# taqu/cpprcoder

Hardware: AMD Instinct MI355X
Metric: MB/s encode+decode per GPU on 64 KiB blocks; ratio vs CPU ref (higher is better)
Workload: dtype u32

## Files before the change

cpprcoder_amd/csrc/rcx_api.hip:

```cpp
#include <hip/hip_runtime.h>

#include <cstdio>
#include <cstdlib>
#include <cstring>
#include <new>
#include <vector>

#include "../../include/rcx.h"
#include "rcx_divtab.hpp"
#include "rcx_kernels.hpp"

namespace
{

#define HIP_TRY(expr)                                                                                              \
    do {                                                                                                           \
        hipError_t e_ = (expr);                                                                                    \
        if (e_ != hipSuccess) {                                                                                    \
            if (getenv("RCX_DEBUG")) fprintf(stderr, "rcx: %s failed: %s (%s:%d)\n", #expr, hipGetErrorString(e_), __FILE__, __LINE__); \
            return RCX_E_HIP;                                                                                      \
        }                                                                                                          \
    } while (0)

struct EventPair {
    hipEvent_t a, b;
    int what;
};

inline hipError_t rcx_enter_device(int device)
{
    (void)hipGetLastError();
    return hipSetDevice(device);
}

struct HostPipe;

}

struct rcx_ctx {
    int device = 0;
    int lanes_per_block = 0;
    int wide_wg = -1;
    int enc_variant = 3;
    int enc_lanes = 0;
    int dec_quads = 0;
    int cus = 256;
    bool rans1_lds_set = false;
    bool rans1w_lds_set = false;
    bool rans_track = false;
    u8* slots = nullptr;
    u64 slots_bytes = 0;
    u32* sizes = nullptr;
    u64 sizes_count = 0;
    u32* starts = nullptr;
    u64 starts_count = 0;
    u32* models = nullptr;
    u64 models_bytes = 0;
    u32* redo = nullptr;
    u64 redo_count = 0;
    u32* ties = nullptr;
    u64 ties_count = 0;
    bool bwt_lds_set = false;
    bool bwt_atomic = false;
    DivEntry* divtab = nullptr;
    u32 divtab_block = 0;
    u32* status = nullptr;
    u32* status_host = nullptr;
    u8* h_in = nullptr;
    u64 h_in_bytes = 0;
    u8* h_out = nullptr;
    u64 h_out_bytes = 0;
    u64* h_off = nullptr;
    u64 h_off_count = 0;
    HostPipe* pipe = nullptr;
    bool timing = false;
    std::vector<EventPair> pending;
    std::vector<EventPair> pool;
    double ms[RCX_T_COUNT] = {};
    uint64_t launches[RCX_T_COUNT] = {};
};

namespace
{

struct Timed {
    rcx_ctx* c;
    hipStream_t s;
    EventPair p;
    bool on;
    Timed(rcx_ctx* ctx, hipStream_t st, int what) : c(ctx), s(st), on(ctx->timing)
    {
        if (!on) return;
        if (!c->pool.empty()) {
            p = c->pool.back();
            c->pool.pop_back();
        } else if (hipEventCreate(&p.a) != hipSuccess || hipEventCreate(&p.b) != hipSuccess) {
            on = false;
            return;
        }
        p.what = what;
        (void)hipEventRecord(p.a, s);
    }
    ~Timed()
    {
        if (!on) return;
        (void)hipEventRecord(p.b, s);
        c->pending.push_back(p);
    }
};

int grow(void** p, u64* have, u64 want)
{
    if (*have >= want) return RCX_OK;
    if (*p) (void)hipFree(*p);
    *p = nullptr;
    *have = 0;
    if (hipMalloc(p, want) != hipSuccess) return RCX_E_NOMEM;
    *have = want;
    return RCX_OK;
}

__global__ void rcx_divtab_k(DivEntry* __restrict__ tab, u64 entries)
{
    const u64 i = (u64)blockIdx.x * blockDim.x + threadIdx.x;
    if (i < entries) tab[i] = rcx_make_div_entry((u32)(256 + i));
}

int ensure_divtab(rcx_ctx* c, u32 block)
{
    if (c->divtab && c->divtab_block >= block) return RCX_OK;
    u32 cover = 1u << 16;
    while (cover < block) cover <<= 1;
    const u64 entries = (u64)cover + 2 * RCX_STAGE;
    if (c->divtab) (void)hipFree(c->divtab);
    c->divtab = nullptr;
    c->divtab_block = 0;
    if (hipMalloc(reinterpret_cast<void**>(&c->divtab), entries * sizeof(DivEntry)) != hipSuccess) return RCX_E_NOMEM;
    hipLaunchKernelGGL(rcx_divtab_k, dim3((u32)((entries + 255) / 256)), dim3(256), 0, nullptr, c->divtab, entries);
    if (hipGetLastError() != hipSuccess || hipDeviceSynchronize() != hipSuccess) return RCX_E_HIP;
    c->divtab_block = cover;
    return RCX_OK;
}

bool block_ok(uint32_t block) { return block >= RCX_MIN_BLOCK && block <= RCX_MAX_BLOCK; }

bool wide_workgroups(const rcx_ctx* c, u64 nblocks)
{
    (void)nblocks;
    return c->wide_wg != 0;
}

int decode_lanes(const rcx_ctx* c, u64 nblocks)
{
    (void)nblocks;
    return c->lanes_per_block ? c->lanes_per_block : 4;
}

u32 pow2_at_least(u64 x)
{
    u32 p = 1;
    while (p < x) p <<= 1;
    return p;
}
u32 encode_lanes(const rcx_ctx* c, u64 nblocks)
{
    if (c->enc_lanes) return (u32)c->enc_lanes;
    const u32 want = pow2_at_least((nblocks + c->cus - 1) / c->cus);
    return want > RCX_LANES ? RCX_LANES : want;
}
u32 decode_quads(const rcx_ctx* c, u64 nblocks)
{
    if (c->dec_quads) return (u32)c->dec_quads;
    const u64 simds = 4ull * c->cus;
    const u32 want = pow2_at_least((nblocks + simds - 1) / simds);
    return want > RCX_QUAD_BLOCKS ? RCX_QUAD_BLOCKS : want;
}

int ensure_redo(rcx_ctx* c, u64 nblocks)
{
    u64 bytes = c->redo_count * sizeof(u32);
    const int r = grow(reinterpret_cast<void**>(&c->redo), &bytes, (nblocks + 1) * sizeof(u32));
    c->redo_count = r == RCX_OK ? bytes / sizeof(u32) : 0;
    return r;
}

struct ScratchRange {
    u64 first = 0;
    bool packed = false;
};
struct ScratchView {
    u8* slots;
// ... 319 lines not shown
        if ((r = ensure_redo(c, nblocks)) != RCX_OK) return r;
    }
    return decode_range(c, coder, d_comp, comp_size, d_offsets, nblocks, block, n, d_dst, s, ScratchRange{});
}

}

namespace
{

int decode_range(rcx_ctx* c, int coder, const void* d_comp, u64 comp_size, const u64* d_offsets, u64 nblocks, u32 block, u64 n, void* d_dst,
                 hipStream_t s, ScratchRange rg)
{
    u32* const redo = c->redo ? c->redo + rg.first : nullptr;
    if (is_rans(coder)) {
        Timed t(c, s, RCX_T_DECODE);
        const u64 per_wg = 4 * RCX_RANS_BLOCKS;
        const u32 grid = (u32)((nblocks + per_wg - 1) / per_wg);
        if (coder == RCX_CODER_RANS8)
            hipLaunchKernelGGL(rcx_dec_rans8_k<4>, dim3(grid), dim3(256), 0, s, static_cast<const u8*>(d_comp), (u64)comp_size, d_offsets, nblocks,
                               block, n, static_cast<u8*>(d_dst), c->status);
        else {
            const u32 quads = rg.packed ? RCX_QUAD_BLOCKS : decode_quads(c, nblocks);
            const u64 per_wg1 = (u64)quads * RCX_QUAD_DEC_WAVES;
            const u32 grid1 = (u32)((nblocks + per_wg1 - 1) / per_wg1);
            hipLaunchKernelGGL(rcx_dec_rans1_quad_k<RCX_QUAD_DEC_WAVES>, dim3(grid1), dim3(64 * RCX_QUAD_DEC_WAVES), 0, s,
                               static_cast<const u8*>(d_comp), (u64)comp_size, d_offsets, nblocks, block, n, static_cast<u8*>(d_dst), c->status,
                               quads, c->rans_track ? c->status + 2 : static_cast<u32*>(nullptr));
        }
        return hipGetLastError() == hipSuccess ? RCX_OK : RCX_E_HIP;
    }
    const bool quad = coder == RCX_CODER_ADAPTIVE && decode_lanes(c, nblocks) == 4;
    const bool squad = coder == RCX_CODER_STATIC && decode_lanes(c, nblocks) != 1;
    {
        Timed t(c, s, RCX_T_DECODE);
        if (coder == RCX_CODER_STATIC && decode_lanes(c, nblocks) != 1) {
            const u32 quads = rg.packed ? RCX_QUAD_BLOCKS : decode_quads(c, nblocks);
            const u64 per_wg = (u64)quads * RCX_QUAD_DEC_WAVES;
            const u32 grid = (u32)((nblocks + per_wg - 1) / per_wg);
            hipLaunchKernelGGL(rcx_dec_static_quad_k<RCX_QUAD_DEC_WAVES>, dim3(grid), dim3(64 * RCX_QUAD_DEC_WAVES), 0, s,
                               static_cast<const u8*>(d_comp), (u64)comp_size, d_offsets, nblocks, block, n, static_cast<u8*>(d_dst), c->status,
                               redo, quads);
        } else if (coder == RCX_CODER_STATIC) {
            const u32 grid = (u32)((nblocks + RCX_LANES - 1) / RCX_LANES);
            hipLaunchKernelGGL(rcx_dec_static_k<false>, dim3(grid), dim3(64), 0, s, static_cast<const u8*>(d_comp), (u64)comp_size, d_offsets, nblocks,
                               block, n, static_cast<u8*>(d_dst), c->status, static_cast<u32*>(nullptr),
                               static_cast<const u32*>(nullptr));
        } else if (decode_lanes(c, nblocks) == 4) {
            const u32 quads = rg.packed ? RCX_QUAD_BLOCKS : decode_quads(c, nblocks);
            if (wide_workgroups(c, nblocks)) {
                const u64 per_wg = (u64)quads * RCX_QUAD_DEC_WAVES;
                const u32 grid = (u32)((nblocks + per_wg - 1) / per_wg);
                hipLaunchKernelGGL(rcx_dec_quad_k<RCX_QUAD_DEC_WAVES>, dim3(grid), dim3(64 * RCX_QUAD_DEC_WAVES), 0, s,
                                   static_cast<const u8*>(d_comp), (u64)comp_size, d_offsets, nblocks, block, n, static_cast<u8*>(d_dst), c->divtab,
                                   c->status, redo, quads);
            } else {
                const u32 grid = (u32)((nblocks + quads - 1) / quads);
                hipLaunchKernelGGL(rcx_dec_quad_k<1>, dim3(grid), dim3(64), 0, s, static_cast<const u8*>(d_comp), (u64)comp_size, d_offsets, nblocks,
                                   block, n, static_cast<u8*>(d_dst), c->divtab, c->status, redo, quads);
            }
#if defined(RCX_WITH_VARIANTS)
        } else if (decode_lanes(c, nblocks) == 8) {
            if (wide_workgroups(c, nblocks)) {
                const u64 per_wg = RCX_OCT_BLOCKS * RCX_OCT_DEC_WAVES;
                const u32 grid = (u32)((nblocks + per_wg - 1) / per_wg);
                hipLaunchKernelGGL(rcx_dec_oct_k<RCX_OCT_DEC_WAVES>, dim3(grid), dim3(64 * RCX_OCT_DEC_WAVES), 0, s,
                                   static_cast<const u8*>(d_comp), (u64)comp_size, d_offsets, nblocks, block, n, static_cast<u8*>(d_dst), c->divtab,
                                   c->status);
            } else {
                const u32 grid = (u32)((nblocks + RCX_OCT_BLOCKS - 1) / RCX_OCT_BLOCKS);
                hipLaunchKernelGGL(rcx_dec_oct_k<1>, dim3(grid), dim3(64), 0, s, static_cast<const u8*>(d_comp), (u64)comp_size, d_offsets, nblocks,
                                   block, n, static_cast<u8*>(d_dst), c->divtab, c->status);
            }
#endif
        } else {
            const u32 grid = (u32)((nblocks + RCX_LANES - 1) / RCX_LANES);
            hipLaunchKernelGGL(rcx_dec_adaptive_k<false>, dim3(grid), dim3(64), 0, s, static_cast<const u8*>(d_comp), (u64)comp_size, d_offsets,
                               nblocks, block, n, static_cast<u8*>(d_dst), c->divtab, c->status, static_cast<u32*>(nullptr),
                               static_cast<const u32*>(nullptr));
        }
        if (quad) {
            const u32 grid = (u32)((nblocks + RCX_LANES - 1) / RCX_LANES);
            hipLaunchKernelGGL(rcx_dec_adaptive_k<false>, dim3(grid), dim3(64), 0, s, static_cast<const u8*>(d_comp), (u64)comp_size, d_offsets,
                               nblocks, block, n, static_cast<u8*>(d_dst), c->divtab, c->status, static_cast<u32*>(nullptr),
                               static_cast<const u32*>(redo));
        }
        if (squad) {
            const u32 grid = (u32)((nblocks + RCX_LANES - 1) / RCX_LANES);
            hipLaunchKernelGGL(rcx_dec_static_k<false>, dim3(grid), dim3(64), 0, s, static_cast<const u8*>(d_comp), (u64)comp_size, d_offsets, nblocks,
                               block, n, static_cast<u8*>(d_dst), c->status, static_cast<u32*>(nullptr), static_cast<const u32*>(redo));
        }
    }
    return hipGetLastError() == hipSuccess ? RCX_OK : RCX_E_HIP;
}

}

extern "C" {

int rcx_encode_blocks(rcx_ctx* c, int coder, const uint8_t* src, uint64_t n, uint32_t block,
                      uint8_t* dst, uint64_t dst_cap, uint64_t* dst_size, uint64_t* offsets)
{
    if (!c || !block_ok(block) || !dst_size || (n && (!src || !dst))) return RCX_E_ARG;
    HIP_TRY(rcx_enter_device(c->device));
    *dst_size = 0;
    if (!coder_ok(coder)) return RCX_E_ARG;
    const u64 nblocks = rcx_block_count(n, block);
    if (nblocks > 0x7FFFFFFFull) return RCX_E_ARG;
    const u64 bound = rcx_encode_bound_for(coder, n, block);
    const u64 cb = host_chunk_blocks(block, false, nblocks);
    const u64 chunks = (nblocks + cb - 1) / cb;
    int r = grow(reinterpret_cast<void**>(&c->h_in), &c->h_in_bytes, n + 64);
// ... 317 lines not shown
            hipLaunchKernelGGL(rcx_dec_static_quad_k<RCX_QUAD_DEC_WAVES>, dim3(1), dim3(64 * RCX_QUAD_DEC_WAVES), 0, nullptr, c->h_in, (u64)comp_size,
                               c->h_off, (u64)1, block, count, c->h_out, c->status, c->redo, 1u);
            if (hipGetLastError() != hipSuccess) return RCX_E_HIP;
            u32 marked = 0;
            const int fast = rcx_ctx_sync_status(c, nullptr, nullptr);
            HIP_TRY(hipMemcpy(&marked, c->redo, sizeof(u32), hipMemcpyDeviceToHost));
            if (fast == RCX_OK && marked == 0) {
                HIP_TRY(hipMemcpy(dst, c->h_out, count, hipMemcpyDeviceToHost));
                *dst_size = count;
                return RCX_OK;
            }
        }
        hipLaunchKernelGGL(rcx_dec_static_k<true>, dim3(1), dim3(64), 0, nullptr, c->h_in, (u64)comp_size, c->h_off, (u64)1, block, count, c->h_out,
                           c->status, c->status + 2, static_cast<const u32*>(nullptr));
        if (hipGetLastError() != hipSuccess) return RCX_E_HIP;
        HIP_TRY(hipMemcpy(c->status_host, c->status, 4 * sizeof(u32), hipMemcpyDeviceToHost));
        const u32 short_at = c->status_host[2];
        const u64 produced = short_at < count ? short_at : count;
        if (produced) HIP_TRY(hipMemcpy(dst, c->h_out, produced, hipMemcpyDeviceToHost));
        *dst_size = produced;
        return short_at < count ? RCX_ERROR : RCX_OK;
    }
    if (comp_size < 8) {
        if (request_size) *request_size = 8;
        return RCX_PENDING;
    }
    const u32 declared = (u32)comp[0] | ((u32)comp[1] << 8) | ((u32)comp[2] << 16) | ((u32)comp[3] << 24);
    const u64 cap16 = sink_capacity;
    const u64 want = declared ? declared : 1;
    const u64 count = want < cap16 ? want : cap16;
    if (count > RCX_MAX_STREAM) return RCX_E_ARG;
    if (count == 0) {
        if (request_size) *request_size = declared;
        return RCX_PENDING;
    }
    const u32 block = count < RCX_MIN_BLOCK ? RCX_MIN_BLOCK : (u32)count;
    const bool longer = count > RCX_MAX_BLOCK;
    int r = longer ? RCX_OK : ensure_divtab(c, block);
    if (r != RCX_OK) return r;
    r = grow(reinterpret_cast<void**>(&c->h_in), &c->h_in_bytes, comp_size + 64);
    if (r != RCX_OK) return r;
    r = grow(reinterpret_cast<void**>(&c->h_out), &c->h_out_bytes, count + 64);
    if (r != RCX_OK) return r;
    u64 off_bytes = c->h_off_count * sizeof(u64);
    r = grow(reinterpret_cast<void**>(&c->h_off), &off_bytes, 2 * sizeof(u64));
    if (r != RCX_OK) return r;
    c->h_off_count = off_bytes / sizeof(u64);
    const u64 offs[2] = {0, comp_size};
    HIP_TRY(hipMemcpy(c->h_in, comp, comp_size, hipMemcpyHostToDevice));
    HIP_TRY(hipMemcpy(c->h_off, offs, sizeof(offs), hipMemcpyHostToDevice));
    if (!longer && count == declared && count >= RCX_MIN_BLOCK && decode_lanes(c, 1) == 4) {
        if ((r = ensure_redo(c, 1)) != RCX_OK) return r;
        hipLaunchKernelGGL(rcx_dec_quad_k<RCX_QUAD_DEC_WAVES>, dim3(1), dim3(64 * RCX_QUAD_DEC_WAVES), 0, nullptr, c->h_in, (u64)comp_size, c->h_off,
                           (u64)1, block, count, c->h_out, c->divtab, c->status, c->redo, 1u);
        if (hipGetLastError() != hipSuccess) return RCX_E_HIP;
        u32 marked = 0;
        const int fast = rcx_ctx_sync_status(c, nullptr, nullptr);
        HIP_TRY(hipMemcpy(&marked, c->redo, sizeof(u32), hipMemcpyDeviceToHost));
        if (fast == RCX_OK && marked == 0) {
            HIP_TRY(hipMemcpy(dst, c->h_out, count, hipMemcpyDeviceToHost));
            *dst_size = count;
            return RCX_OK;
        }
    }
    if (longer)
        hipLaunchKernelGGL((rcx_dec_adaptive_k<true, true>), dim3(1), dim3(64), 0, nullptr, c->h_in, (u64)comp_size, c->h_off, (u64)1, block, count, c->h_out,
                           c->divtab, c->status, c->status + 2, static_cast<const u32*>(nullptr));
    else
        hipLaunchKernelGGL((rcx_dec_adaptive_k<true, false>), dim3(1), dim3(64), 0, nullptr, c->h_in, (u64)comp_size, c->h_off, (u64)1, block, count, c->h_out,
                           c->divtab, c->status, c->status + 2, static_cast<const u32*>(nullptr));
    if (hipGetLastError() != hipSuccess) return RCX_E_HIP;
    HIP_TRY(hipMemcpy(c->status_host, c->status, 4 * sizeof(u32), hipMemcpyDeviceToHost));
    const u32 short_at = c->status_host[2];
    u64 produced = count;
    int result = RCX_OK;
    if (short_at != 0xFFFFFFFFu && short_at < count) {
        produced = short_at;
        result = RCX_PENDING;
    } else if (want > cap16) {
        result = RCX_PENDING;
    }
    if (result == RCX_PENDING && request_size) *request_size = declared - (u32)produced;
    if (produced) HIP_TRY(hipMemcpy(dst, c->h_out, produced, hipMemcpyDeviceToHost));
    *dst_size = produced;
    return result;
}

struct rcx_dstream {
    rcx_ctx* ctx = nullptr;
    RcxDState* state = nullptr;
    u8* in = nullptr;
    u64 in_base = 0;
    u64 in_bytes = 0, in_cap = 0;
    u64 consumed = 0;
    u8* out = nullptr;
    u32* result = nullptr;
    u32* result_host = nullptr;
    bool finished = false;
    u32 declared = 0, produced = 0;
};
#define RCX_DSTREAM_CHUNK (1u << 20)

int rcx_dstream_create(rcx_ctx* c, rcx_dstream** out)
{
    if (!c || !out) return RCX_E_ARG;
    *out = nullptr;
    HIP_TRY(rcx_enter_device(c->device));
// ... 507 lines not shown
```

cpprcoder_amd/csrc/rcx_oct.hpp:

```cpp
#pragma once

template <int CTRL>
__device__ __forceinline__ u32 rcx_dpp(u32 x)
{
    return (u32)__builtin_amdgcn_update_dpp(0, (int)x, CTRL, 0xF, 0xF, true);
}
__device__ __forceinline__ u32 rcx_oct_sum(u32 x)
{
    x += rcx_dpp<0xB1>(x);
    x += rcx_dpp<0x4E>(x);
    x += rcx_dpp<0x141>(x);
    return x;
}
__device__ __forceinline__ u32 rcx_oct_excl_scan(u32 x, u32 m1, u32 m2, u32 m4)
{
    u32 tot = x, pre = 0, o;
    o = rcx_dpp<0xB1>(tot);
    pre += o & m1;
    tot += o;
    o = rcx_dpp<0x4E>(tot);
    pre += o & m2;
    tot += o;
    o = rcx_dpp<0x141>(tot);
    pre += o & m4;
    return pre;
}

#define RCX_MC_CHUNK 16
#define RCX_MC_THREADS 256
#define RCX_MC_RING_U4 (2 * RCX_MC_CHUNK * RCX_LANES)
#define RCX_MC_LDS_U4 (RCX_LDS_U4 + RCX_MC_RING_U4)

__device__ __forceinline__ void rcx_lds_barrier()
{
    asm volatile("s_waitcnt lgkmcnt(0)\n\ts_barrier" ::: "memory");
}

#if defined(RCX_STAMP)
static __device__ unsigned long long rcx_stamp_out[16];
#define rcx_stamp_wait stamp_wait_
#endif
#define RCX_QUAD_BLOCKS 16
#define RCX_QUAD_STAGE 16
#define RCX_QUAD_GROUP_BYTES 4352
#define RCX_QUAD_RING_BYTES 144
#define RCX_QUAD_LDS_BYTES (RCX_QUAD_STAGE * 16 + 4 * RCX_QUAD_GROUP_BYTES + RCX_QUAD_BLOCKS * RCX_QUAD_RING_BYTES)

typedef u32 RcxV4 __attribute__((ext_vector_type(4)));
typedef __attribute__((address_space(3))) RcxV4 RcxLdsV4;
typedef __attribute__((address_space(3))) u32 RcxLdsU32;
typedef RcxV4 RcxDivQv;
typedef RcxLdsV4 RcxLdsDivQ;

struct alignas(16) DivQ {
    u32 mul, st;
    u64 add;
};

__device__ __forceinline__ u32 rcx_quad_sum(u32 x)
{
    x += rcx_dpp<0xB1>(x);
    x += rcx_dpp<0x4E>(x);
    return x;
}
__device__ __forceinline__ u32 rcx_umin(u32 a, u32 b) { return a < b ? a : b; }
__device__ __forceinline__ u32 rcx_umax(u32 a, u32 b) { return a > b ? a : b; }
__device__ __forceinline__ u32 rcx_quad_min(u32 x)
{
    x = rcx_umin(x, rcx_dpp<0xB1>(x));
    x = rcx_umin(x, rcx_dpp<0x4E>(x));
    return x;
}
__device__ __forceinline__ u32 rcx_quad_max(u32 x)
{
    x = rcx_umax(x, rcx_dpp<0xB1>(x));
    x = rcx_umax(x, rcx_dpp<0x4E>(x));
    return x;
}
__device__ __forceinline__ u32 rcx_quad_or(u32 x)
{
    x |= rcx_dpp<0xB1>(x);
    x |= rcx_dpp<0x4E>(x);
    return x;
}
__device__ __forceinline__ u32 rcx_quad_excl_scan(u32 x, u32 m1, u32 m2)
{
    u32 o = rcx_dpp<0xB1>(x);
    u32 pre = o & m1;
    const u32 tot = x + o;
    o = rcx_dpp<0x4E>(tot);
    pre += o & m2;
    return pre;
}

#if !defined(RCX_TOPUP_PIECES)
#define RCX_TOPUP_PIECES 1
#endif
struct QuadInput {
    u32 low, range;
    u32 bp8;
    u32 w0, w1;
    u32 n4;
    u32* ring;
    U4* skipped;
    u32 wr;
    u32 nfit;
    U4 pendA, pendB;
    const u8* origin;
    u32 last_off;
    u32 body8;
// ... 26 lines not shown
        origin = body - ((uintptr_t)body & 15);
        last_off = (u32)(stream_end - 1 - origin) & ~15u;
        wr = 0;
        for (u32 r = 0; r < 6; ++r) ring_put(load16(16 * r), true);
        nfit = 0;
        pendA.x = pendA.y = pendA.z = pendA.w = 0;
        pendB = pendA;
        body8 = 8u * (u32)(body - origin);
        bp8 = body8;
        fetch_pair();
        n4 = rcx_bswap(rcx_funnel_shr(w1, w0, bp8));
        return declared;
    }
    __device__ __forceinline__ void idle(const u8* anywhere, u32* block_ring, U4* scratch16)
    {
        skipped = scratch16;
        low = 0;
        range = 0x01000000u;
        ring = block_ring;
        origin = anywhere - ((uintptr_t)anywhere & 15);
        last_off = 0;
        wr = 24;
        nfit = 0;
        pendA.x = pendA.y = pendA.z = pendA.w = 0;
        pendB = pendA;
        body8 = bp8 = 0;
        w0 = w1 = n4 = 0;
    }
    __device__ __forceinline__ void topup()
    {
        ring_put(pendA, nfit >= 1);
#if RCX_TOPUP_PIECES > 1
        ring_put(pendB, nfit >= 2);
#endif
        const u32 rd = bp8 >> 5;
        if (rcx_any(wr - rd < 14u)) {
            asm volatile("" ::: "memory");
            while (__any(wr - rd <= 20u)) ring_put(load16(4 * wr), wr - rd <= 20u);
        }
        const u32 room = (rd + RCX_RING_DW - wr) >> 2;
        nfit = room < (u32)RCX_TOPUP_PIECES ? room : (u32)RCX_TOPUP_PIECES;
        pendA = load16(4 * wr);
#if RCX_TOPUP_PIECES > 1
        pendB = load16(4 * wr + 16);
#endif
    }
    __device__ __forceinline__ u64 taken() const { return 8 + (u64)((bp8 - body8) >> 3); }
};

#define RCX_QUAD_DEC_WAVES 4
template <int WAVES>
__global__ __launch_bounds__(64 * WAVES) void rcx_dec_quad_k(const u8* __restrict__ comp, u64 comp_size, const u64* __restrict__ offsets,
                                                             u64 nblocks, u32 block, u64 n, u8* __restrict__ dst,
                                                             const DivEntry* __restrict__ divtab, u32* status,
                                                             u32* __restrict__ redo, u32 quads_used)
{
    __shared__ __attribute__((aligned(256))) u8 lds_all[WAVES * RCX_QUAD_LDS_BYTES];
    const u32 lane = threadIdx.x & 63u;
    const u32 wave_in_wg = __builtin_amdgcn_readfirstlane(threadIdx.x >> 6);
    u8* lds = lds_all + wave_in_wg * RCX_QUAD_LDS_BYTES;
    const u32 j = lane & 3u, quad = lane >> 2;
    const bool in_use = quad < quads_used;
    const u64 blk = ((u64)blockIdx.x * WAVES + wave_in_wg) * quads_used + (quad & (quads_used - 1u));
    bool live = blk < nblocks;
    const u64 at = live ? blk * (u64)block : 0;
    u32 len = live ? (u32)((n - at) < (u64)block ? (n - at) : (u64)block) : 0u;

    DivQ* stage = reinterpret_cast<DivQ*>(lds);
    const u32 group = 2u * (quad >> 3) + ((0x96u >> (quad & 7u)) & 1u), quarter = (quad & 7u) >> 1;
    u8* mine = lds + RCX_QUAD_STAGE * 16 + group * RCX_QUAD_GROUP_BYTES + quarter * 64;
    U4* leaves = reinterpret_cast<U4*>(mine) + j;
    U4* parked = reinterpret_cast<U4*>(mine + 16 * 256);
    u32* block_ring = reinterpret_cast<u32*>(lds + RCX_QUAD_STAGE * 16 + 4 * RCX_QUAD_GROUP_BYTES + quad * RCX_QUAD_RING_BYTES);
    {
        U4 v;
        v.x = v.y = v.z = v.w = 1;
#pragma unroll
        for (u32 q = 0; q < 17; ++q) leaves[q * 16] = v;
    }
    u32 U1 = 64u * j + 16, U2 = U1 + 16, U3 = U1 + 32, U4_ = U1 + 48;
    const u32 T0 = 4u * j;
    const u32 m1 = (j & 1u) ? ~0u : 0u, m2 = (j & 2u) ? ~0u : 0u;

    QuadInput in;
    u64 stream_len = 0;
    if (live) {
        const u64 s0 = offsets[blk], s1 = offsets[blk + 1];
        stream_len = s1 - s0;
        if (s1 < s0 || s1 > comp_size || stream_len < 9) {
            if (j == 0 && in_use) rcx_flag(status, RCX_ST_CORRUPT, blk);
            live = false;
            len = 0;
        } else {
            const u32 declared = in.begin(comp + s0, comp + s1, block_ring, parked + 3);
            if (declared != len) {
                if (j == 0 && in_use) rcx_flag(status, RCX_ST_CORRUPT, blk);
                live = false;
                len = 0;
            }
        }
    }
    if (!live) in.idle(comp, block_ring, parked + 3);

    const u32 maxlen = rcx_wave_max(len);
    u8* out = dst + at;
    u32 fast_end;
    {
        u32 mine = live ? (len & ~15u) : 0xFFFFFFF0u;
        if (live && (reinterpret_cast<uintptr_t>(out) & 15u) != 0) mine = 0;
#pragma unroll
        for (int o = 32; o > 0; o >>= 1) {
            const u32 other = (u32)__shfl_xor((int)mine, o, 64);
            mine = mine < other ? mine : other;
        }
        fast_end = mine == 0xFFFFFFF0u ? 0u : mine;
    }
    const bool leader = live && in_use && j == 0;

    const u32 T0p3 = T0 + 3;
    const u32 leaves_lds = (u32)reinterpret_cast<uintptr_t>(leaves);
    const u32 ring_lds = (u32)reinterpret_cast<uintptr_t>(block_ring);
#if defined(RCX_STAMP_DEC)
#define RCX_QUAD_STAMP(i) if (stamp_now_) stamp_t_[stamp_at_ + (i)] = __builtin_amdgcn_s_memtime();
#else
#define RCX_QUAD_STAMP(i)
#endif
#define RCX_QP1 "quad_perm:[1,0,3,2] row_mask:0xf bank_mask:0xf bound_ctrl:1\n\t"
#define RCX_QP2 "quad_perm:[2,3,0,1] row_mask:0xf bank_mask:0xf bound_ctrl:1\n\t"
    u32 p_sym_ = 0, p_la_ = leaves_lds;
    u64 p_own_ = 0;
#define RCX_QD_PREV_A_0 "s_nop 1\n\t"
#define RCX_QD_PREV_A_1 "v_cndmask_b32_e64 %[pown], 0, 1, %[pc]\n\t"                                                \
                        "v_and_b32 %[pad], 3, %[psym]\n\t"                                                         \
                        "v_lshl_add_u32 %[pad], %[pad], 2, %[pla]\n\t"
#define RCX_QD_PREV_S_0
#define RCX_QD_PREV_S_1 "\n\tv_cndmask_b32_e64 %[pye], 0, %[psym], %[pc]\n\t"                                       \
                        "v_lshl_or_b32 %[pword], %[pye], %[psh], %[pword]"
#define RCX_QUAD_DEC_SYMBOL(K, HP, PWORD, PSHIFT)                                                           \
    {                                                                                                      \
            \
        const u32 k8_ = rcx_clz(in.range) & 0x18u;                                                         \
        in.low = (u32)((((u64)in.low << 32) | in.n4) << k8_ >> 32);                                        \
        in.range <<= k8_;                                                                                  \
        const DivQ k_ = (K);                                                                               \
        const u32 t_ = (u32)(((u64)in.range * k_.mul + k_.add) >> 32) >> (k_.st & 31u);           \
              \
        const u32 a1_ = rcx_mul24(U1, t_), a2_ = rcx_mul24(U2, t_), a3_ = rcx_mul24(U3, t_);               \
        const u32 a4_ = rcx_mul24(U4_, t_);                                                                \
        u32 node_, rem_, ro_, la_, x1_, x2_, x3_, x4_, pown_, pad_, pye_;                                  \
        u64 c1_, c2_, c3_, c4_, cz_;                                                                       \
        asm volatile("v_sub_co_u32_e64 %[x1], %[c1], %[low], %[a1]\n\t"                                    \
                     "v_sub_co_u32_e64 %[x2], %[c2], %[low], %[a2]\n\t"                                    \
                     "v_sub_co_u32_e64 %[x3], %[c3], %[low], %[a3]\n\t"                                    \
                     "v_sub_co_u32_e64 %[x4], %[c4], %[low], %[a4]\n\t"                                    \
                     "v_subb_co_u32_e64 %[nd], %[cz], 4, 0, %[c1]\n\t"  \
                     "v_subb_co_u32_e64 %[nd], %[cz], %[nd], 0, %[c2]\n\t"                                 \
                     "v_subb_co_u32_e64 %[nd], %[cz], %[nd], 0, %[c3]\n\t"                                 \
                     "v_subb_co_u32_e64 %[nd], %[cz], %[nd], 0, %[c4]\n\t"                                 \
                     RCX_QD_PREV_A_##HP                                                                    \
                     : [nd] "=&v"(node_), [x1] "=&v"(x1_), [x2] "=&v"(x2_), [x3] "=&v"(x3_), [x4] "=&v"(x4_), \
                       [c1] "=&s"(c1_), [c2] "=&s"(c2_), [c3] "=&s"(c3_), [c4] "=&s"(c4_), [cz] "=&s"(cz_), \
                       [pown] "=&v"(pown_), [pad] "=&v"(pad_)                                              \
                     : [low] "v"(in.low), [a1] "v"(a1_), [a2] "v"(a2_), [a3] "v"(a3_), [a4] "v"(a4_),      \
                       [pc] "s"(p_own_), [psym] "v"(p_sym_), [pla] "v"(p_la_));                            \
        if (HP) (void)__hip_atomic_fetch_add(reinterpret_cast<RcxLdsU32*>(pad_), pown_, __ATOMIC_RELAXED, __HIP_MEMORY_SCOPE_WAVEFRONT);  \
        asm volatile("v_add_u32_dpp %[nd], %[nd], %[nd] " RCX_QP1                                          \
                     "v_add_u32 %[bp], %[bp], %[k8]\n\t"                 \
                     "v_bfe_u32 %[ro], %[bp], 5, 5\n\t"                 \
                     "v_lshl_add_u32 %[ro], %[ro], 2, %[rb]"  \
                     : [nd] "+v"(node_), [ro] "=&v"(ro_), [bp] "+v"(in.bp8)                                 \
                     : [k8] "v"(k8_), [rb] "v"(ring_lds));                                                 \
        {                                                                                                  \
            const RcxLdsU32* at_ = reinterpret_cast<const RcxLdsU32*>(ro_);  \
            in.w0 = at_[0];                                                                                \
            in.w1 = at_[1];                                                                                \
        }                                                                                                  \
        __builtin_amdgcn_sched_barrier(0);                                                                 \
        asm volatile("v_add_u32_dpp %[nd], %[nd], %[nd] " RCX_QP2                                          \
                     "v_lshl_add_u32 %[la], %[nd], 8, %[lvb]"  \
                     : [nd] "+v"(node_), [la] "=&v"(la_)                                                    \
                     : [lvb] "v"(leaves_lds));                                                             \
                                                              \
        RCX_QUAD_STAMP(0);                                                                                 \
        const RcxV4 l_ = *reinterpret_cast<const RcxLdsV4*>(la_);                                          \
        __builtin_amdgcn_sched_barrier(0);                                                                 \
                    \
        u32 sb_;                                                                                           \
        asm volatile("v_min3_u32 %[rm], %[x1], %[x2], %[x3]\n\t"                                           \
                     "v_min3_u32 %[rm], %[rm], %[x4], %[low]\n\t"                                          \
                     "v_addc_co_u32_e64 %[u1], %[c1], 0, %[u1], %[c1]\n\t"                                 \
                     "v_addc_co_u32_e64 %[u2], %[c2], 0, %[u2], %[c2]\n\t"                                 \
                     "v_min_u32_dpp %[rm], %[rm], %[rm] " RCX_QP1                                          \
                     "v_addc_co_u32_e64 %[u3], %[c3], 0, %[u3], %[c3]\n\t"                                 \
                     "v_addc_co_u32_e64 %[u4], %[c4], 0, %[u4], %[c4]\n\t"                                 \
                     "v_min_u32_dpp %[rm], %[rm], %[rm] " RCX_QP2                                          \
                     "v_lshl_add_u32 %[sb], %[n], 4, %[t0p3]"  \
                     RCX_QD_PREV_S_##HP                                                                    \
                     : [u1] "+v"(U1), [u2] "+v"(U2), [u3] "+v"(U3), [u4] "+v"(U4_), [rm] "=&v"(rem_),       \
// ... 5 lines not shown
        asm volatile("v_mul_u32_u24 %[qa], %[lx], %[t]\n\t"       \
                     "v_mad_u32_u24 %[qb], %[ly], %[t], %[qa]\n\t"       \
                     "v_mad_u32_u24 %[qc], %[lz], %[t], %[qb]\n\t"                                         \
                     "v_mad_u32_u24 %[qe], %[lw], %[t], %[qc]\n\t"                                         \
                     "v_alignbit_b32 %[n4], %[w1], %[w0], %[bp]\n\t"  \
                     "v_perm_b32 %[n4], %[n4], %[n4], %[swap]\n\t"  \
                     "v_add_u32_dpp %[tot], %[qe], %[qe] " RCX_QP1  \
                     "v_and_b32_dpp %[pre], %[qe], %[m1] " RCX_QP1                                         \
                     "v_sub_u32 %[d2], %[rem], %[pre]\n\t"                                                 \
                     "v_and_b32_dpp %[o2], %[tot], %[m2] " RCX_QP2                                         \
                     "v_sub_u32 %[d2], %[d2], %[o2]\n\t"      \
                     "v_sub_co_u32_e64 %[ya], %[c1], %[d2], %[qa]\n\t"                                     \
                     "v_sub_co_u32_e64 %[yb], %[c2], %[d2], %[qb]\n\t"                                     \
                     "v_sub_co_u32_e64 %[yc], %[c3], %[d2], %[qc]\n\t"                                     \
                     "v_sub_co_u32_e64 %[ye], %[own], %[d2], %[qe]\n\t"  \
                     "v_min3_u32 %[lo], %[d2], %[ya], %[yb]\n\t"                                           \
                     "v_max3_u32 %[hi], %[ya], %[yb], %[yc]\n\t"                                           \
                     "v_min_u32 %[lo], %[lo], %[yc]\n\t"                                                   \
                     "v_max_u32 %[hi], %[hi], %[ye]\n\t"                                                   \
                     "v_subb_co_u32_e64 %[sym], %[c1], %[sb], 0, %[c1]\n\t"                                \
                     "v_min_u32_dpp %[lo], %[lo], %[lo] " RCX_QP1                                          \
                     "v_subb_co_u32_e64 %[sym], %[c2], %[sym], 0, %[c2]\n\t"                               \
                     "v_max_u32_dpp %[hi], %[hi], %[hi] " RCX_QP1                                          \
                     "v_subb_co_u32_e64 %[sym], %[c3], %[sym], 0, %[c3]\n\t"                               \
                     "v_min_u32_dpp %[lo], %[lo], %[lo] " RCX_QP2                                          \
                     "v_max_u32_dpp %[hi], %[hi], %[hi] " RCX_QP2                                          \
                     "v_sub_u32 %[rg], %[lo], %[hi]"                                                       \
                     : [lo] "=&v"(lo_), [rg] "=&v"(rg_), [sym] "=&v"(p_sym_), [own] "=&s"(p_own_), [n4] "=&v"(in.n4), \
                       [qa] "=&v"(qa_), [qb] "=&v"(qb_), [qc] "=&v"(qc_),                                   \
                       [qe] "=&v"(qe_), [tot] "=&v"(tot_), [pre] "=&v"(pre_), [o2] "=&v"(o2_), [d2] "=&v"(d2_), \
                       [ya] "=&v"(ya_), [yb] "=&v"(yb_), [yc] "=&v"(yc_), [ye] "=&v"(ye_), [hi] "=&v"(hi_),  \
                       [c1] "=&s"(c1_), [c2] "=&s"(c2_), [c3] "=&s"(c3_)                                   \
                     : [lx] "v"(l_.x), [ly] "v"(l_.y), [lz] "v"(l_.z), [lw] "v"(l_.w), [t] "v"(t_),        \
                       [rem] "v"(rem_), [m1] "v"(m1), [m2] "v"(m2), [sb] "v"(sb_),                         \
                       [w0] "v"(in.w0), [w1] "v"(in.w1), [bp] "v"(in.bp8), [swap] "s"(0x00010203u));       \
        RCX_QUAD_STAMP(1);                                                                                 \
        in.low = lo_;                                                                            \
        in.range = rg_;                                                                          \
        p_la_ = la_;                                                                                       \
    }
#define RCX_QUAD_DEC_FINISH(WORD, SHIFT)                                                                    \
    {                                                                                                      \
        u32 pown_, pad_, pye_;                                                                             \
        asm volatile("v_cndmask_b32_e64 %[pown], 0, 1, %[pc]\n\t"                                          \
                     "v_and_b32 %[pad], 3, %[psym]\n\t"                                                    \
                     "v_cndmask_b32_e64 %[pye], 0, %[psym], %[pc]\n\t"                                     \
                     "v_lshl_add_u32 %[pad], %[pad], 2, %[pla]\n\t"                                        \
                     "v_lshl_or_b32 %[pword], %[pye], %[psh], %[pword]"                                    \
                     : [pown] "=&v"(pown_), [pad] "=&v"(pad_), [pye] "=&v"(pye_), [pword] "+v"(WORD)        \
                     : [pc] "s"(p_own_), [psym] "v"(p_sym_), [pla] "v"(p_la_), [psh] "n"(SHIFT));          \
        (void)__hip_atomic_fetch_add(reinterpret_cast<RcxLdsU32*>(pad_), pown_, __ATOMIC_RELAXED, __HIP_MEMORY_SCOPE_WAVEFRONT);  \
    }

    DivEntry ahead = divtab[lane % RCX_QUAD_STAGE];
#define RCX_QUAD_STAGE_PUT()                                                                               \
    {                                                                                                      \
        DivQ q_;                                                                                           \
        q_.mul = ahead.mul;                                                                                \
        q_.st = (ahead.total << 5) | ahead.shift;                                                          \
        q_.add = ahead.add;                                                                                \
        stage[lane % RCX_QUAD_STAGE] = q_;                           \
    }
#define RCX_QUAD_STAGE_GET(I0) ahead = divtab[(I0) + RCX_QUAD_STAGE + lane % RCX_QUAD_STAGE];
    {
        U4 o_last;
        o_last.x = o_last.y = o_last.z = o_last.w = 0;
#if defined(RCX_STAMP_DEC)
        unsigned long long stamp_sum_[4] = {0, 0, 0, 0};
#endif
        for (u32 i0 = 0; i0 < fast_end; i0 += 16) {
            RCX_QUAD_STAGE_PUT();
            in.topup();
            RCX_QUAD_STAGE_GET(i0);
            const u32 g = (i0 >> 4) & 3u;
            if (g == 0 && i0 != 0 && leader) {
                U4* o4 = reinterpret_cast<U4*>(out + (i0 - 64));
                const U4 p0 = parked[0], p1 = parked[1], p2 = parked[2];
                o4[0] = p0;
                o4[1] = p1;
                o4[2] = p2;
                o4[3] = o_last;
            }
            u32 w0_ = 0, w1_ = 0, w2_ = 0, w3_ = 0;
            DivQ k_next = stage[0];
#if defined(RCX_STAMP_DEC)
            unsigned long long stamp_t_[4] = {0, 0, 0, 0};
#define RCX_QUAD_STEP(S, HP, PW)                                 \
    {                                                            \
        const DivQ kk = k_next;                                  \
        if ((S) + 1 < 16) k_next = stage[(S) + 1];               \
        const bool stamp_now_ = (S) == 8 || (S) == 9;            \
        const int stamp_at_ = (S) == 8 ? 0 : 2;                  \
        RCX_QUAD_DEC_SYMBOL(kk, HP, PW, (8 * (((S) + 3) & 3))); \
    }
#else
#define RCX_QUAD_STEP(S, HP, PW)                                 \
    {                                                            \
        const DivQ kk = k_next;                                  \
        if ((S) + 1 < 16) k_next = stage[(S) + 1];               \
        RCX_QUAD_DEC_SYMBOL(kk, HP, PW, (8 * (((S) + 3) & 3))); \
    }
#endif
            RCX_QUAD_STEP(0, 0, w0_) RCX_QUAD_STEP(1, 1, w0_) RCX_QUAD_STEP(2, 1, w0_) RCX_QUAD_STEP(3, 1, w0_)
            RCX_QUAD_STEP(4, 1, w0_) RCX_QUAD_STEP(5, 1, w1_) RCX_QUAD_STEP(6, 1, w1_) RCX_QUAD_STEP(7, 1, w1_)
            RCX_QUAD_STEP(8, 1, w1_) RCX_QUAD_STEP(9, 1, w2_) RCX_QUAD_STEP(10, 1, w2_) RCX_QUAD_STEP(11, 1, w2_)
            RCX_QUAD_STEP(12, 1, w2_) RCX_QUAD_STEP(13, 1, w3_) RCX_QUAD_STEP(14, 1, w3_) RCX_QUAD_STEP(15, 1, w3_)
            RCX_QUAD_DEC_FINISH(w3_, 24)
#undef RCX_QUAD_STEP
#if defined(RCX_STAMP_DEC)
            stamp_sum_[0] += stamp_t_[1] - stamp_t_[0];
            stamp_sum_[1] += stamp_t_[2] - stamp_t_[1];
            stamp_sum_[2] += stamp_t_[3] - stamp_t_[2];
            stamp_sum_[3] += 1;
#endif
            U4 o;
            o.x = rcx_quad_or(w0_);
            o.y = rcx_quad_or(w1_);
            o.z = rcx_quad_or(w2_);
            o.w = rcx_quad_or(w3_);
            if (g == 3) o_last = o;
            else parked[g] = o;
        }
#if defined(RCX_STAMP_DEC)
        if (blockIdx.x == 7 && threadIdx.x == 0)
            for (int i_ = 0; i_ < 4; ++i_) rcx_dec_stamp_out[i_] = stamp_sum_[i_];
#endif
        if (leader && fast_end != 0) {
            const u32 groups = ((fast_end - 1) >> 4 & 3u) + 1;
            U4* o4 = reinterpret_cast<U4*>(out + ((fast_end - 1) & ~63u));
            o4[0] = parked[0];
            if (groups > 1) o4[1] = parked[1];
            if (groups > 2) o4[2] = parked[2];
            if (groups > 3) o4[3] = o_last;
        }
    }
    {
        for (u32 i = fast_end; i < maxlen; ++i) {
            if ((i & 15u) == 0) {
                RCX_QUAD_STAGE_PUT();
                in.topup();
                RCX_QUAD_STAGE_GET(i);
            }
            const DivQ k = stage[i % RCX_QUAD_STAGE];
            if (i < len) {
                u32 part = 0;
#if defined(RCX_STAMP_DEC)
                const bool stamp_now_ = false;
                const int stamp_at_ = 0;
                unsigned long long stamp_t_[4];
#endif
                RCX_QUAD_DEC_SYMBOL(k, 0, part, 0);
                RCX_QUAD_DEC_FINISH(part, 0);
                part = rcx_quad_or(part);
                if (leader) out[i] = (u8)part;
            }
        }
    }
#undef RCX_QUAD_DEC_SYMBOL
#undef RCX_QUAD_DEC_FINISH
#undef RCX_QD_PREV_A_0
#undef RCX_QD_PREV_A_1
#undef RCX_QD_PREV_S_0
#undef RCX_QD_PREV_S_1
#undef RCX_QUAD_STAGE_PUT
#undef RCX_QUAD_STAGE_GET
#undef RCX_QP1
#undef RCX_QP2
    const bool marked = live && rcx_quad_or(j == 3 && U4_ != 256u + len ? 1u : 0u) != 0;
    if (leader && !marked && in.taken() > stream_len) rcx_flag(status, RCX_ST_CORRUPT, blk);
    if (leader) redo[blk] = marked ? 1u : 0u;
    else if (j == 0 && in_use && blk < nblocks) redo[blk] = 0;
}

#if !defined(RCX_DRAIN_WAVE)
#define RCX_DRAIN_WAVE 5
#endif
#if RCX_DRAIN_WAVE == 5
#define RCX_MC5_THREADS 384
#define RCX_MC5_ROLE(HW) ((HW) == 1u ? 3u : (HW) == 3u ? 1u : (HW))
#else
#define RCX_MC5_THREADS 320
#define RCX_MC5_ROLE(HW) (HW)
#endif
#if !defined(RCX_RING_PLANAR)
#define RCX_RING_PLANAR 0
#endif
#if !defined(RCX_MODEL_AHEAD)
#define RCX_MODEL_AHEAD 2
#endif
#if !defined(RCX_ARITH_AHEAD)
#define RCX_ARITH_AHEAD 1
#endif
#if RCX_RING_PLANAR
#define RCX_RING_LANE 1
#define RCX_RING_AT(s, f) ((4 * (s) + (f)) * RCX_LANES)
#else
#define RCX_RING_LANE 4
#define RCX_RING_AT(s, f) (4 * (s) * RCX_LANES + (f))
#endif
#define RCX_MC5_RING2_DW (2 * RCX_MC_CHUNK * RCX_LANES)
#define RCX_OUT_RING_WORDS 64
#define RCX_OUT_MARGIN 32
#define RCX_MC5_OUT_DW (RCX_OUT_RING_WORDS * RCX_LANES + 3 * RCX_LANES)
#define RCX_MC5_LDS_U4 (RCX_MC_LDS_U4 + RCX_MC5_RING2_DW / 4 + RCX_LANES / 4 + RCX_MC5_OUT_DW / 4)

struct __attribute__((packed, aligned(4))) RcxU4Unaligned {
    u32 x, y, z, w;
};

__device__ __attribute__((noinline, cold)) u32 rcx_stage_carry(u32* ring_lane, u32 pos, u32 safe_from, u32 extra)
{
    while (extra != 0 && pos > safe_from) {
        --pos;
        u32* w = ring_lane + ((pos >> 2) % RCX_OUT_RING_WORDS) * RCX_LANES;
        const u32 sh = 8u * (pos & 3u);
        const u32 old = *w;
        const u32 v = ((old >> sh) & 0xFFu) + extra;
        *w = (old & ~(0xFFu << sh)) | ((v & 0xFFu) << sh);
// ... 418 lines not shown
```

Before: 69560.

## Replace LDS-staged division table with packed global mul/inc table in quad decoder

Adds a second precomputed table holding each divisor's multiplier and a 0/1 increment flag, packed in groups of 16 so a quad can load four U4 vectors per 16-symbol group. The quad decoder now computes the quotient with __umulhi((range<<k)+inc, mul) >> shift, with the shift derived from clz of the position, instead of a 64-bit multiply-add. The LDS staging area and its per-group store and reload are removed, and loads for the next group are software-pipelined between steps. This trades LDS traffic and 64-bit arithmetic for global/scalar loads held in extra registers, and relies on the increment formulation matching the old add term exactly.

```diff
diff --git a/cpprcoder_amd/csrc/rcx_api.hip b/cpprcoder_amd/csrc/rcx_api.hip
--- a/cpprcoder_amd/csrc/rcx_api.hip
+++ b/cpprcoder_amd/csrc/rcx_api.hip
@@ -63,6 +63,7 @@
     bool bwt_lds_set = false;
     bool bwt_atomic = false;
     DivEntry* divtab = nullptr;
+    u32* divq = nullptr;
     u32 divtab_block = 0;
     u32* status = nullptr;
     u32* status_host = nullptr;
@@ -120,10 +121,16 @@
     return RCX_OK;
 }
 
-__global__ void rcx_divtab_k(DivEntry* __restrict__ tab, u64 entries)
+__global__ void rcx_divtab_k(DivEntry* __restrict__ tab, u32* __restrict__ divq, u64 entries)
 {
     const u64 i = (u64)blockIdx.x * blockDim.x + threadIdx.x;
-    if (i < entries) tab[i] = rcx_make_div_entry((u32)(256 + i));
+    if (i < entries) {
+        const DivEntry e = rcx_make_div_entry((u32)(256 + i));
+        tab[i] = e;
+        u32* g = divq + (i >> 4) * RCX_QUAD_DIVQ_DW + (i & 15u);
+        g[0] = e.mul;
+        g[16] = e.add == 0 ? 0u : 1u;
+    }
 }
 
 int ensure_divtab(rcx_ctx* c, u32 block)
@@ -134,9 +141,11 @@
     const u64 entries = (u64)cover + 2 * RCX_STAGE;
     if (c->divtab) (void)hipFree(c->divtab);
     c->divtab = nullptr;
+    c->divq = nullptr;
     c->divtab_block = 0;
-    if (hipMalloc(reinterpret_cast<void**>(&c->divtab), entries * sizeof(DivEntry)) != hipSuccess) return RCX_E_NOMEM;
-    hipLaunchKernelGGL(rcx_divtab_k, dim3((u32)((entries + 255) / 256)), dim3(256), 0, nullptr, c->divtab, entries);
+    if (hipMalloc(reinterpret_cast<void**>(&c->divtab), entries * (sizeof(DivEntry) + 2 * sizeof(u32))) != hipSuccess) return RCX_E_NOMEM;
+    c->divq = reinterpret_cast<u32*>(c->divtab + entries);
+    hipLaunchKernelGGL(rcx_divtab_k, dim3((u32)((entries + 255) / 256)), dim3(256), 0, nullptr, c->divtab, c->divq, entries);
     if (hipGetLastError() != hipSuccess || hipDeviceSynchronize() != hipSuccess) return RCX_E_HIP;
     c->divtab_block = cover;
     return RCX_OK;
@@ -562,12 +571,12 @@
                 const u64 per_wg = (u64)quads * RCX_QUAD_DEC_WAVES;
                 const u32 grid = (u32)((nblocks + per_wg - 1) / per_wg);
                 hipLaunchKernelGGL(rcx_dec_quad_k<RCX_QUAD_DEC_WAVES>, dim3(grid), dim3(64 * RCX_QUAD_DEC_WAVES), 0, s,
-                                   static_cast<const u8*>(d_comp), (u64)comp_size, d_offsets, nblocks, block, n, static_cast<u8*>(d_dst), c->divtab,
+                                   static_cast<const u8*>(d_comp), (u64)comp_size, d_offsets, nblocks, block, n, static_cast<u8*>(d_dst), c->divq,
                                    c->status, redo, quads);
             } else {
                 const u32 grid = (u32)((nblocks + quads - 1) / quads);
                 hipLaunchKernelGGL(rcx_dec_quad_k<1>, dim3(grid), dim3(64), 0, s, static_cast<const u8*>(d_comp), (u64)comp_size, d_offsets, nblocks,
-                                   block, n, static_cast<u8*>(d_dst), c->divtab, c->status, redo, quads);
+                                   block, n, static_cast<u8*>(d_dst), c->divq, c->status, redo, quads);
             }
 #if defined(RCX_WITH_VARIANTS)
         } else if (decode_lanes(c, nblocks) == 8) {
@@ -991,7 +1000,7 @@
     if (!longer && count == declared && count >= RCX_MIN_BLOCK && decode_lanes(c, 1) == 4) {
         if ((r = ensure_redo(c, 1)) != RCX_OK) return r;
         hipLaunchKernelGGL(rcx_dec_quad_k<RCX_QUAD_DEC_WAVES>, dim3(1), dim3(64 * RCX_QUAD_DEC_WAVES), 0, nullptr, c->h_in, (u64)comp_size, c->h_off,
-                           (u64)1, block, count, c->h_out, c->divtab, c->status, c->redo, 1u);
+                           (u64)1, block, count, c->h_out, c->divq, c->status, c->redo, 1u);
         if (hipGetLastError() != hipSuccess) return RCX_E_HIP;
         u32 marked = 0;
         const int fast = rcx_ctx_sync_status(c, nullptr, nullptr);
diff --git a/cpprcoder_amd/csrc/rcx_oct.hpp b/cpprcoder_amd/csrc/rcx_oct.hpp
--- a/cpprcoder_amd/csrc/rcx_oct.hpp
+++ b/cpprcoder_amd/csrc/rcx_oct.hpp
@@ -41,10 +41,9 @@
 #define rcx_stamp_wait stamp_wait_
 #endif
 #define RCX_QUAD_BLOCKS 16
-#define RCX_QUAD_STAGE 16
 #define RCX_QUAD_GROUP_BYTES 4352
 #define RCX_QUAD_RING_BYTES 144
-#define RCX_QUAD_LDS_BYTES (RCX_QUAD_STAGE * 16 + 4 * RCX_QUAD_GROUP_BYTES + RCX_QUAD_BLOCKS * RCX_QUAD_RING_BYTES)
+#define RCX_QUAD_LDS_BYTES (4 * RCX_QUAD_GROUP_BYTES + RCX_QUAD_BLOCKS * RCX_QUAD_RING_BYTES)
 
 typedef u32 RcxV4 __attribute__((ext_vector_type(4)));
 typedef __attribute__((address_space(3))) RcxV4 RcxLdsV4;
@@ -56,6 +55,8 @@
     u32 mul, st;
     u64 add;
 };
+
+#define RCX_QUAD_DIVQ_DW 32
 
 __device__ __forceinline__ u32 rcx_quad_sum(u32 x)
 {
@@ -188,7 +189,7 @@
 template <int WAVES>
 __global__ __launch_bounds__(64 * WAVES) void rcx_dec_quad_k(const u8* __restrict__ comp, u64 comp_size, const u64* __restrict__ offsets,
                                                              u64 nblocks, u32 block, u64 n, u8* __restrict__ dst,
-                                                             const DivEntry* __restrict__ divtab, u32* status,
+                                                             const u32* __restrict__ divq, u32* status,
                                                              u32* __restrict__ redo, u32 quads_used)
 {
     __shared__ __attribute__((aligned(256))) u8 lds_all[WAVES * RCX_QUAD_LDS_BYTES];
@@ -202,12 +203,11 @@
     const u64 at = live ? blk * (u64)block : 0;
     u32 len = live ? (u32)((n - at) < (u64)block ? (n - at) : (u64)block) : 0u;
 
-    DivQ* stage = reinterpret_cast<DivQ*>(lds);
     const u32 group = 2u * (quad >> 3) + ((0x96u >> (quad & 7u)) & 1u), quarter = (quad & 7u) >> 1;
-    u8* mine = lds + RCX_QUAD_STAGE * 16 + group * RCX_QUAD_GROUP_BYTES + quarter * 64;
+    u8* mine = lds + group * RCX_QUAD_GROUP_BYTES + quarter * 64;
     U4* leaves = reinterpret_cast<U4*>(mine) + j;
     U4* parked = reinterpret_cast<U4*>(mine + 16 * 256);
-    u32* block_ring = reinterpret_cast<u32*>(lds + RCX_QUAD_STAGE * 16 + 4 * RCX_QUAD_GROUP_BYTES + quad * RCX_QUAD_RING_BYTES);
+    u32* block_ring = reinterpret_cast<u32*>(lds + 4 * RCX_QUAD_GROUP_BYTES + quad * RCX_QUAD_RING_BYTES);
     {
         U4 v;
         v.x = v.y = v.z = v.w = 1;
@@ -272,14 +272,13 @@
 #define RCX_QD_PREV_S_0
 #define RCX_QD_PREV_S_1 "\n\tv_cndmask_b32_e64 %[pye], 0, %[psym], %[pc]\n\t"                                       \
                         "v_lshl_or_b32 %[pword], %[pye], %[psh], %[pword]"
-#define RCX_QUAD_DEC_SYMBOL(K, HP, PWORD, PSHIFT)                                                           \
+#define RCX_QUAD_DEC_SYMBOL(MUL, INC, SH, HP, PWORD, PSHIFT)                                               \
     {                                                                                                      \
             \
         const u32 k8_ = rcx_clz(in.range) & 0x18u;                                                         \
         in.low = (u32)((((u64)in.low << 32) | in.n4) << k8_ >> 32);                                        \
-        in.range <<= k8_;                                                                                  \
-        const DivQ k_ = (K);                                                                               \
-        const u32 t_ = (u32)(((u64)in.range * k_.mul + k_.add) >> 32) >> (k_.st & 31u);           \
+                  \
+        const u32 t_ = __umulhi((in.range << k8_) + (INC), (MUL)) >> (SH);                                 \
               \
         const u32 a1_ = rcx_mul24(U1, t_), a2_ = rcx_mul24(U2, t_), a3_ = rcx_mul24(U3, t_);               \
         const u32 a4_ = rcx_mul24(U4_, t_);                                                                \
@@ -391,26 +390,30 @@
         (void)__hip_atomic_fetch_add(reinterpret_cast<RcxLdsU32*>(pad_), pown_, __ATOMIC_RELAXED, __HIP_MEMORY_SCOPE_WAVEFRONT);  \
     }
 
-    DivEntry ahead = divtab[lane % RCX_QUAD_STAGE];
-#define RCX_QUAD_STAGE_PUT()                                                                               \
+#if defined(RCX_QUAD_DIV_SMEM)
+    const u32* dq_ = divq;
+#else
+    u32 vz_;
+    asm volatile("v_mov_b32 %0, 0" : "=v"(vz_));
+    const u32* dq_ = divq + vz_;
+#endif
+#define RCX_QUAD_DIVQ_LOAD(G, Q)                                                                             \
     {                                                                                                      \
-        DivQ q_;                                                                                           \
-        q_.mul = ahead.mul;                                                                                \
-        q_.st = (ahead.total << 5) | ahead.shift;                                                          \
-        q_.add = ahead.add;                                                                                \
-        stage[lane % RCX_QUAD_STAGE] = q_;                           \
-    }
-#define RCX_QUAD_STAGE_GET(I0) ahead = divtab[(I0) + RCX_QUAD_STAGE + lane % RCX_QUAD_STAGE];
+        __builtin_amdgcn_sched_barrier(0);                                                                 \
+        dm##Q = reinterpret_cast<const U4*>(dq_ + (G) * RCX_QUAD_DIVQ_DW)[Q];                              \
+        di##Q = reinterpret_cast<const U4*>(dq_ + (G) * RCX_QUAD_DIVQ_DW + 16)[Q];                         \
+    }
+#define RCX_QUAD_U4_AT(V, C) ((C) == 0 ? (V).x : (C) == 1 ? (V).y : (C) == 2 ? (V).z : (V).w)
     {
         U4 o_last;
         o_last.x = o_last.y = o_last.z = o_last.w = 0;
 #if defined(RCX_STAMP_DEC)
         unsigned long long stamp_sum_[4] = {0, 0, 0, 0};
 #endif
+        U4 dm0, dm1, dm2, dm3, di0, di1, di2, di3;
+        RCX_QUAD_DIVQ_LOAD(0u, 0) RCX_QUAD_DIVQ_LOAD(0u, 1) RCX_QUAD_DIVQ_LOAD(0u, 2) RCX_QUAD_DIVQ_LOAD(0u, 3)
         for (u32 i0 = 0; i0 < fast_end; i0 += 16) {
-            RCX_QUAD_STAGE_PUT();
             in.topup();
-            RCX_QUAD_STAGE_GET(i0);
             const u32 g = (i0 >> 4) & 3u;
             if (g == 0 && i0 != 0 && leader) {
                 U4* o4 = reinterpret_cast<U4*>(out + (i0 - 64));
@@ -421,29 +424,29 @@
                 o4[3] = o_last;
             }
             u32 w0_ = 0, w1_ = 0, w2_ = 0, w3_ = 0;
-            DivQ k_next = stage[0];
+            const u32 sh_ = 31u - (u32)__builtin_clz(256u + i0);
+            const u32 gn_ = (i0 >> 4) + 1u;
 #if defined(RCX_STAMP_DEC)
             unsigned long long stamp_t_[4] = {0, 0, 0, 0};
-#define RCX_QUAD_STEP(S, HP, PW)                                 \
-    {                                                            \
-        const DivQ kk = k_next;                                  \
-        if ((S) + 1 < 16) k_next = stage[(S) + 1];               \
-        const bool stamp_now_ = (S) == 8 || (S) == 9;            \
-        const int stamp_at_ = (S) == 8 ? 0 : 2;                  \
-        RCX_QUAD_DEC_SYMBOL(kk, HP, PW, (8 * (((S) + 3) & 3))); \
+#define RCX_QUAD_STEP(S, Q, HP, PW)                                                                           \
+    {                                                                                                        \
+        const bool stamp_now_ = (S) == 8 || (S) == 9;                                                        \
+        const int stamp_at_ = (S) == 8 ? 0 : 2;                                                              \
+        RCX_QUAD_DEC_SYMBOL(RCX_QUAD_U4_AT(dm##Q, (S) & 3), RCX_QUAD_U4_AT(di##Q, (S) & 3), sh_, HP, PW,     \
+                            (8 * (((S) + 3) & 3)));                                                          \
     }
 #else
-#define RCX_QUAD_STEP(S, HP, PW)                                 \
-    {                                                            \
-        const DivQ kk = k_next;                                  \
-        if ((S) + 1 < 16) k_next = stage[(S) + 1];               \
-        RCX_QUAD_DEC_SYMBOL(kk, HP, PW, (8 * (((S) + 3) & 3))); \
-    }
-#endif
-            RCX_QUAD_STEP(0, 0, w0_) RCX_QUAD_STEP(1, 1, w0_) RCX_QUAD_STEP(2, 1, w0_) RCX_QUAD_STEP(3, 1, w0_)
-            RCX_QUAD_STEP(4, 1, w0_) RCX_QUAD_STEP(5, 1, w1_) RCX_QUAD_STEP(6, 1, w1_) RCX_QUAD_STEP(7, 1, w1_)
-            RCX_QUAD_STEP(8, 1, w1_) RCX_QUAD_STEP(9, 1, w2_) RCX_QUAD_STEP(10, 1, w2_) RCX_QUAD_STEP(11, 1, w2_)
-            RCX_QUAD_STEP(12, 1, w2_) RCX_QUAD_STEP(13, 1, w3_) RCX_QUAD_STEP(14, 1, w3_) RCX_QUAD_STEP(15, 1, w3_)
+#define RCX_QUAD_STEP(S, Q, HP, PW)                                                                           \
+    RCX_QUAD_DEC_SYMBOL(RCX_QUAD_U4_AT(dm##Q, (S) & 3), RCX_QUAD_U4_AT(di##Q, (S) & 3), sh_, HP, PW, (8 * (((S) + 3) & 3)));
+#endif
+            RCX_QUAD_STEP(0, 0, 0, w0_) RCX_QUAD_STEP(1, 0, 1, w0_) RCX_QUAD_STEP(2, 0, 1, w0_) RCX_QUAD_STEP(3, 0, 1, w0_)
+            RCX_QUAD_DIVQ_LOAD(gn_, 0)
+            RCX_QUAD_STEP(4, 1, 1, w0_) RCX_QUAD_STEP(5, 1, 1, w1_) RCX_QUAD_STEP(6, 1, 1, w1_) RCX_QUAD_STEP(7, 1, 1, w1_)
+            RCX_QUAD_DIVQ_LOAD(gn_, 1)
+            RCX_QUAD_STEP(8, 2, 1, w1_) RCX_QUAD_STEP(9, 2, 1, w2_) RCX_QUAD_STEP(10, 2, 1, w2_) RCX_QUAD_STEP(11, 2, 1, w2_)
+            RCX_QUAD_DIVQ_LOAD(gn_, 2)
+            RCX_QUAD_STEP(12, 3, 1, w2_) RCX_QUAD_STEP(13, 3, 1, w3_) RCX_QUAD_STEP(14, 3, 1, w3_) RCX_QUAD_STEP(15, 3, 1, w3_)
+            RCX_QUAD_DIVQ_LOAD(gn_, 3)
             RCX_QUAD_DEC_FINISH(w3_, 24)
 #undef RCX_QUAD_STEP
 #if defined(RCX_STAMP_DEC)
@@ -474,13 +477,18 @@
         }
     }
     {
+        u32 mul_n_, inc_n_;
+#define RCX_QUAD_DIVQ_ENTRY(I)                                                                              \
+    {                                                                                                      \
+        const u32* e_ = divq + ((I) >> 4) * RCX_QUAD_DIVQ_DW + ((I) & 15u);                                 \
+        mul_n_ = e_[0];                                                                                    \
+        inc_n_ = e_[16];                                                                                   \
+    }
+        RCX_QUAD_DIVQ_ENTRY(fast_end);
         for (u32 i = fast_end; i < maxlen; ++i) {
-            if ((i & 15u) == 0) {
-                RCX_QUAD_STAGE_PUT();
-                in.topup();
-                RCX_QUAD_STAGE_GET(i);
-            }
-            const DivQ k = stage[i % RCX_QUAD_STAGE];
+            if ((i & 15u) == 0) in.topup();
+            const u32 mul_ = mul_n_, inc_ = inc_n_, sh_ = 31u - (u32)__builtin_clz(256u + i);
+            RCX_QUAD_DIVQ_ENTRY(i + 1u);
             if (i < len) {
                 u32 part = 0;
 #if defined(RCX_STAMP_DEC)
@@ -488,7 +496,7 @@
                 const int stamp_at_ = 0;
                 unsigned long long stamp_t_[4];
 #endif
-                RCX_QUAD_DEC_SYMBOL(k, 0, part, 0);
+                RCX_QUAD_DEC_SYMBOL(mul_, inc_, sh_, 0, part, 0);
                 RCX_QUAD_DEC_FINISH(part, 0);
                 part = rcx_quad_or(part);
                 if (leader) out[i] = (u8)part;
@@ -501,8 +509,9 @@
 #undef RCX_QD_PREV_A_1
 #undef RCX_QD_PREV_S_0
 #undef RCX_QD_PREV_S_1
-#undef RCX_QUAD_STAGE_PUT
-#undef RCX_QUAD_STAGE_GET
+#undef RCX_QUAD_DIVQ_LOAD
+#undef RCX_QUAD_DIVQ_ENTRY
+#undef RCX_QUAD_U4_AT
 #undef RCX_QP1
 #undef RCX_QP2
     const bool marked = live && rcx_quad_or(j == 3 && U4_ != 256u + len ? 1u : 0u) != 0;
```

After: 70870 (median of 6 runs). +1.9%, better.
